# lucidrains/egnn-pytorch

Hardware: AMD Instinct MI355X
Metric: EGNN.forward graphs/sec (higher is better)
Workload: dtype f32; 1 GPU; EGNN(dim=512) masked k-NN (k=32) B=64/GPU N=1024 fp32; graphs_per_gpu=64, nodes=1024, neighbors=32, layers=1, global_batch=64, mask=all-true, parallelism=batch-shard x1 (no data-path collective)

## Files before the change

egnn_pytorch_amd/csrc/edge_pw.hip:

```cpp
#include <type_traits>
#include "egnn_common.h"
#include "egnn_lds_dma.h"

namespace {

typedef _Float16 f16x8 __attribute__((ext_vector_type(8)));
typedef _Float16 f16x4 __attribute__((ext_vector_type(4)));
typedef _Float16 f16x2 __attribute__((ext_vector_type(2)));
typedef float f32x2v __attribute__((ext_vector_type(2)));
typedef uint32_t u32x2 __attribute__((ext_vector_type(2)));
typedef uint32_t u32x4v __attribute__((ext_vector_type(4)));

#ifndef EGNN_PW_WGS
#define EGNN_PW_WGS 5
#endif
#ifndef EGNN_PW_SKIP_MASKED
#define EGNN_PW_SKIP_MASKED 1
#endif
#ifndef EGNN_PW_RESID4
#define EGNN_PW_RESID4 1
#endif

constexpr int PW_THREADS = 256;
constexpr int PW_WAVES = 4;
#ifndef EGNN_PW_EARLY_W
#define EGNN_PW_EARLY_W 1
#endif
#ifndef EGNN_PW_PRIO
#define EGNN_PW_PRIO 0
#endif
#ifndef EGNN_PW_HC
#define EGNN_PW_HC 64
#endif
#ifndef EGNN_PW_ABL
#define EGNN_PW_ABL 0
#endif
constexpr int PW_HC = EGNN_PW_HC;
constexpr int PW_XLD = 32;
constexpr int PW_W2S = 0;
constexpr int PW_WST = PW_W2S + 2 * PW_HC * 64;
constexpr int PW_XCH = PW_WST + 2 * PW_HC * 16;
constexpr int PW_REC = PW_XCH + PW_WAVES * 32 * PW_XLD * 4;
constexpr int PW_SCR = PW_REC + PW_WAVES * 2 * 512;
constexpr int PW_LDS = PW_SCR + PW_WAVES * 256;

__device__ __forceinline__ uint32_t pw_pack_h2(_Float16 a, _Float16 b)
{
    const f16x2 v = {a, b};
    return __builtin_bit_cast(uint32_t, v);
}

template <typename T>
__device__ __forceinline__ T pw_opaque(T v)
{
    asm volatile("" : "+s"(v));
    return v;
}

__device__ __forceinline__ uint32_t lds_addr_of(const void* p)
{
    return __builtin_amdgcn_readfirstlane((uint32_t)(size_t)(__attribute__((address_space(3))) char*)(char*)p);
}

typedef const __attribute__((address_space(4))) egnn_edge_args* pw_args_ptr;
__device__ __forceinline__ pw_args_ptr pw_args()
{
    pw_args_ptr a = (pw_args_ptr)__builtin_amdgcn_kernarg_segment_ptr();
    asm volatile("" : "+s"(a));
    return a;
}

template <bool MULTI>
__global__ __launch_bounds__(PW_THREADS, EGNN_PW_WGS) void edge_pw_kernel(const egnn_edge_args p)
{
    __shared__ __attribute__((aligned(16))) char smem[PW_LDS];

    const int tid = threadIdx.x;
    const int lane = tid & 63;
    const int wave = __builtin_amdgcn_readfirstlane(tid >> 6);
    const int e = lane & 15;
    const int g = lane >> 4;
    const int N = p.N, K = p.K;
    const int R = MULTI ? (K >> 5) : 1;
    const int T = p.B * N;

    const int ngroups = (T + PW_WAVES - 1) / PW_WAVES;
    const int nper = (int)(gridDim.x >> 3);
    const int xcd = (int)(blockIdx.x & 7), wi = (int)(blockIdx.x >> 3);
    const int gq = ngroups >> 3, grem = ngroups & 7;
    const int gstart = xcd * gq + (xcd < grem ? xcd : grem);
    const int gcount = gq + (xcd < grem ? 1 : 0);
    if (wi >= gcount) return;
    const int mygroups = (gcount - wi + nper - 1) / nper;
    const int total_rounds = mygroups * R;

    _Float16* const w2s = reinterpret_cast<_Float16*>(smem + PW_W2S);
    char* const wst = smem + PW_WST;
    float* const xch = reinterpret_cast<float*>(smem + PW_XCH) + wave * (32 * PW_XLD);
    char* const recb = smem + PW_REC + wave * 1024;
    float* const scr = reinterpret_cast<float*>(smem + PW_SCR) + wave * 64;
    const uint32_t xch_lds = lds_addr_of(xch);
    const uint32_t rec_lds = lds_addr_of(recb);

    const int Hp = p.Hp;
    const int nchunks = (Hp + PW_HC - 1) / PW_HC;
#if defined(EGNN_PW_NO_HALF_TAIL) && EGNN_PW_NO_HALF_TAIL
    const bool half_tail = false;
#else
    const bool half_tail = Hp - p.H >= 16;
#endif

    const char* const w2h_g = reinterpret_cast<const char*>(p.W2h);
    const char* const wst_g = reinterpret_cast<const char*>(p.Wst);
    const uint32_t lane16 = (uint32_t)lane * 16u;
    auto stage = [&](int c, int slot) {
        const int c0s = c * PW_HC;
        const int hcs = (Hp - c0s) < PW_HC ? (Hp - c0s) : PW_HC;
        const char* src = w2h_g + (size_t)c0s * 64;
        char* dst = reinterpret_cast<char*>(w2s) + slot * (PW_HC * 64);
        for (int pc = wave; pc < hcs / 16; pc += PW_WAVES) lds_dma16_s(src + pc * 1024, lane16, dst + pc * 1024);
        if (wave == 0) {
            const int tbytes = hcs * 16;
            for (int o = 0; o < tbytes; o += 1024)
                if ((int)lane16 + o < tbytes) lds_dma16_s(wst_g + (size_t)c0s * 16 + o, lane16, wst + slot * (PW_HC * 16) + o);
        }
    };
    auto rec_dma = [&](int tau, int r, int buf) {
        const pw_args_ptr a = pw_args();
        const u32x4s slot_words = make_rsrc_words(a->slots, (uint32_t)((size_t)a->B * a->N * a->K * 16));
        const uint32_t soff = ((uint32_t)tau * (uint32_t)a->K + 32u * (uint32_t)r) * 16u;
        if (lane < 32) gather_dma16(slot_words, (uint32_t)lane * 16u, soff, rec_lds + (uint32_t)buf * 512u);
    };
    auto node_of = [&](int kg) { return (gstart + wi + kg * nper) * PW_WAVES + wave; };
    int zero_v = 0;
    asm volatile("" : "+v"(zero_v));
    auto row_of = [&](int tau) {
        const pw_args_ptr a = pw_args();
        return a->order ? a->order[tau + zero_v] : tau % a->N;
    };

    const float* xr[2];
#pragma unroll
    for (int hb = 0; hb < 2; ++hb) xr[hb] = xch + e * PW_XLD + 4 * ((4 * hb + g) ^ ((e >> 1) & 7));
    const char* const tl = wst + (e * 4 + (g ^ ((e >> 2) & 2))) * 4;
    constexpr int tstep = 16 * 4 * 4;
#if EGNN_PW_RESID4
    f16x4 neg_identity;
#pragma unroll
    for (int u = 0; u < 4; ++u) neg_identity[u] = ((lane & 3) == u) ? (_Float16)-1.f : (_Float16)0.f;
#else
    f16x4 neg_identity;
#pragma unroll
    for (int u = 0; u < 4; ++u) neg_identity[u] = (e == 4 * g + u) ? (_Float16)-1.f : (_Float16)0.f;
#endif
#if defined(EGNN_PW_STAGGER) && EGNN_PW_STAGGER
    for (int q = 0; q < ((wi / 32) % EGNN_PW_WGS) * EGNN_PW_STAGGER; ++q) __builtin_amdgcn_s_sleep(127);
#endif
    stage(0, 0);
    int tau_next = node_of(0);
    bool live_next = tau_next < T;
    if (!live_next) tau_next = T - 1;
    rec_dma(tau_next, 0, 0);
    int i_next_v = row_of(tau_next);
    int ring = 0;

    f32x4 nms = f32x4{0.f, 0.f, 0.f, 0.f};
    float ncs[4] = {0.f, 0.f, 0.f, 0.f};

    int kg = 0, r = 0;
    for (int rho = 0; rho < total_rounds; ++rho) {
        const pw_args_ptr pa = pw_args();
        const int64_t ldp = pa->ldp;
        const int tau = tau_next;
        const bool live = live_next;
        const int b = tau / N;
        const size_t bN = (size_t)b * N;
        const int i = __builtin_amdgcn_readfirstlane(i_next_v);
        const uint32_t prow_bytes = (uint32_t)((size_t)N * ldp * 4);
        const __amdgpu_buffer_rsrc_t pi_rsrc = __builtin_amdgcn_make_buffer_rsrc(const_cast<float*>(pa->Pi + bN * ldp), 0, prow_bytes, 0x00020000);
        const u32x4s pj_words = make_rsrc_words(pa->Pj + bN * ldp, prow_bytes);
        const int cur = rho & 1;
        const char* const rb = recb + cur * 512;

        asm volatile("s_waitcnt vmcnt(0)" ::: "memory");
        __builtin_amdgcn_wave_barrier();
        uint32_t goff[4];
#pragma unroll
        for (int qq = 0; qq < 4; ++qq) {
            const uint32_t j2 = *reinterpret_cast<const uint32_t*>(rb + (8 * qq + (lane >> 3)) * 16) & 0x3fffffffu;
            const uint32_t gchunk = (uint32_t)(((lane & 7) ^ ((4 * qq + (lane >> 4)) & 7)) * 16);
            goff[qq] = (uint32_t)((size_t)j2 * ldp * 4) + gchunk;
        }
        u32x4v rec[2];
#pragma unroll
        for (int t = 0; t < 2; ++t) rec[t] = *reinterpret_cast<const u32x4v*>(rb + (16 * t + e) * 16);
#pragma unroll
        for (int qq = 0; qq < 4; ++qq) gather_dma16(pj_words, goff[qq], 0u, xch_lds + qq * 1024);
        const uint32_t piw = (uint32_t)(((size_t)i * ldp + e) * 4);
        uint32_t piv[2];
        piv[0] = buf_load1(pi_rsrc, piw, 0);
        piv[1] = buf_load1(pi_rsrc, piw, 64);
        if (rho + 1 < total_rounds) {
            if (r + 1 == R) {
                tau_next = node_of(kg + 1);
                live_next = tau_next < T;
                if (!live_next) tau_next = T - 1;
                i_next_v = row_of(tau_next);
                rec_dma(tau_next, 0, cur ^ 1);
            } else {
                rec_dma(tau, r + 1, cur ^ 1);
            }
        }

        u32x2 bq[2];
        bool fm[2];
        const int gq_ = g + pw_opaque(0);
        const uint32_t gm0 = gq_ == 0 ? 0xffffffffu : 0u, gm1 = gq_ == 1 ? 0xffffffffu : 0u, gm2 = gq_ == 2 ? 0xffffffffu : 0u;
#pragma unroll
        for (int t = 0; t < 2; ++t) {
            const uint32_t r0 = rec[t][0], r1 = rec[t][1], r2 = rec[t][2], r3 = rec[t][3];
            const float d = egnn_sqdist_rel(__uint_as_float(r1), __uint_as_float(r2), __uint_as_float(r3));
            float val = d * pa->ws_inv_scale;
            egnn_flag_range(pa->status, live && fabsf(val) >= 6.0e7f && fabsf(val) < __builtin_inff(), EGNN_RANGE_SCALAR);
            if (fabsf(val) >= 6.0e7f) val = __builtin_nanf("");
            const _Float16 s1 = (_Float16)(val * (1.0f / 1024.0f));
            const float rem = val - (float)s1 * 1024.0f;
            const _Float16 rh = (_Float16)rem;
            const _Float16 rl = (_Float16)(rem - (float)rh);
            u32x2 bw;
            bw[0] = 0x3c003c00u & gm0;
            bw[1] = (pw_pack_h2(s1, s1) & gm0) | (pw_pack_h2(rh, rh) & gm1) | (pw_pack_h2(rl, (_Float16)0.f) & gm2);
            bq[t] = bw;
            fm[t] = live && (r0 >> 31) != 0u;
        }

        f32x4 acc[2];
#pragma unroll
        for (int t = 0; t < 2; ++t) acc[t] = f32x4{0.f, 0.f, 0.f, 0.f};
#if EGNN_PW_SKIP_MASKED
        const bool skip_round = pa->U_out == nullptr && __builtin_amdgcn_ballot_w64(fm[0] || fm[1]) == 0ull;
        const bool skip_group = skip_round && ((__builtin_amdgcn_readfirstlane(*reinterpret_cast<const int*>(rb)) >> 30) & 1) != 0;
#else
        constexpr bool skip_round = false, skip_group = false;
#endif

        const bool last_round = rho + 1 == total_rounds;
        auto step = [&](auto half_tag, const int c, const int st, const int slot, const int hoff, const _Float16* w2c, const char* tlc) {
            constexpr bool HALF = decltype(half_tag)::value;
            constexpr int NHB = HALF ? 1 : 2;
            const bool more = hoff + 32 < Hp;
            const int hnext = more ? hoff + 32 : hoff;
            f32x4 x[2][2];
            uint32_t pivn[2];
#if EGNN_PW_EARLY_W
            u32x2 a0[2];
#pragma unroll
            for (int hb = 0; hb < NHB; ++hb)
                a0[hb] = u32x2{0u, *reinterpret_cast<const uint32_t*>(tlc + st * 2 * tstep + hb * tstep)};
            const f16x8 whi = *reinterpret_cast<const f16x8*>(w2c + ((st * 2 + 0) * 64 + lane) * 8);
            const f16x8 wlo = *reinterpret_cast<const f16x8*>(w2c + ((st * 2 + 1) * 64 + lane) * 8);
#endif
#if EGNN_PW_ABL & 2
#pragma unroll
            for (int t = 0; t < 2; ++t)
#pragma unroll
                for (int hb = 0; hb < NHB; ++hb) { x[t][hb] = acc[t] * 0.25f; asm volatile("" : "+v"(x[t][hb])); }
#else
            asm volatile("" ::: "memory");
            __builtin_amdgcn_s_waitcnt(0x0F70);
            asm volatile("" ::: "memory");
            __builtin_amdgcn_wave_barrier();
#pragma unroll
            for (int t = 0; t < 2; ++t)
#pragma unroll
                for (int hb = 0; hb < NHB; ++hb) x[t][hb] = *reinterpret_cast<const f32x4*>(xr[hb] + t * 16 * PW_XLD);
            asm volatile("" ::: "memory");
            __builtin_amdgcn_s_waitcnt(0xC07F);
            asm volatile("" ::: "memory");
            __builtin_amdgcn_wave_barrier();
#endif
            if (!HALF) {
#if EGNN_PW_ABL & 256
                pivn[0] = piv[0]; pivn[1] = piv[1];
#else
                pivn[0] = buf_load1(pi_rsrc, piw, hnext * 4);
                pivn[1] = buf_load1(pi_rsrc, piw, hnext * 4 + 64);
#endif
            }
#if !(EGNN_PW_ABL & 128)
            if (st == 0) {
                if (c + 1 < nchunks) stage(c + 1, slot ^ 1);
                else if (!last_round) stage(0, slot ^ 1);
            }
#endif
#if !(EGNN_PW_ABL & 1)
            if (more) {
#pragma unroll
                for (int qq = 0; qq < 4; ++qq) gather_dma16(pj_words, goff[qq], (uint32_t)(hnext * 4), xch_lds + qq * 1024);
            }
#endif

#if EGNN_PW_EARLY_W
#pragma unroll
            for (int hb = 0; hb < NHB; ++hb) a0[hb][0] = piv[hb];
#else
            u32x2 a0[2];
#pragma unroll
            for (int hb = 0; hb < NHB; ++hb)
                a0[hb] = u32x2{piv[hb], *reinterpret_cast<const uint32_t*>(tlc + st * 2 * tstep + hb * tstep)};
            const f16x8 whi = *reinterpret_cast<const f16x8*>(w2c + ((st * 2 + 0) * 64 + lane) * 8);
            const f16x8 wlo = *reinterpret_cast<const f16x8*>(w2c + ((st * 2 + 1) * 64 + lane) * 8);
#endif
            if (!HALF) {
                piv[0] = pivn[0];
                piv[1] = pivn[1];
            }
#pragma unroll
            for (int t = 0; t < 2; ++t)
#pragma unroll
                for (int hb = 0; hb < NHB; ++hb) {
#if EGNN_PW_ABL & 4
                    asm volatile("" :: "v"(a0[hb]), "v"(bq[t]));
#else
                    x[t][hb] = __builtin_amdgcn_mfma_f32_16x16x16f16(__builtin_bit_cast(f16x4, a0[hb]), __builtin_bit_cast(f16x4, bq[t]), x[t][hb], 0, 0, 0);
#endif
                }
#pragma unroll
            for (int t = 0; t < 2; ++t) {
                f16x8 bhi, blo;
#pragma unroll
                for (int u = 0; u < 8; ++u) { bhi[u] = (_Float16)0.f; blo[u] = (_Float16)0.f; }
#pragma unroll
                for (int hb = 0; hb < NHB; ++hb) {
                    f32x4 a4;
#pragma unroll
                    for (int u = 0; u < 4; ++u) {
                        const float y = x[t][hb][u];
#if EGNN_PW_ABL & 32
                        float h = y;
#else
                        float h = y * __builtin_amdgcn_rcpf(1.0f + __builtin_amdgcn_exp2f(y));
#endif
                        asm("" : "+v"(h));
                        a4[u] = h;
                    }
#if EGNN_PW_ABL & 512
                    const f16x2 h01 = __builtin_bit_cast(f16x2, a4[0]), h23 = __builtin_bit_cast(f16x2, a4[2]);
#else
                    const f16x2 h01 = __builtin_convertvector((f32x2v){a4[0], a4[1]}, f16x2);
                    const f16x2 h23 = __builtin_convertvector((f32x2v){a4[2], a4[3]}, f16x2);
#endif
                    const f16x4 hi4 = {h01[0], h01[1], h23[0], h23[1]};
#if EGNN_PW_ABL & 8
                    const f32x4 l4 = a4;
                    asm volatile("" :: "v"(neg_identity));
#elif EGNN_PW_RESID4
                    const f32x4 l4 = __builtin_amdgcn_mfma_f32_4x4x4f16(neg_identity, hi4, a4, 0, 0, 0);
#else
                    const f32x4 l4 = __builtin_amdgcn_mfma_f32_16x16x16f16(neg_identity, hi4, a4, 0, 0, 0);
#endif
#if EGNN_PW_ABL & 512
                    const f16x2 l01 = __builtin_bit_cast(f16x2, l4[1]), l23 = __builtin_bit_cast(f16x2, l4[3]);
#else
                    const f16x2 l01 = __builtin_bit_cast(f16x2, __builtin_amdgcn_cvt_pkrtz(l4[0], l4[1]));
                    const f16x2 l23 = __builtin_bit_cast(f16x2, __builtin_amdgcn_cvt_pkrtz(l4[2], l4[3]));
#endif
                    bhi[4 * hb + 0] = h01[0]; bhi[4 * hb + 1] = h01[1]; bhi[4 * hb + 2] = h23[0]; bhi[4 * hb + 3] = h23[1];
                    blo[4 * hb + 0] = l01[0]; blo[4 * hb + 1] = l01[1]; blo[4 * hb + 2] = l23[0]; blo[4 * hb + 3] = l23[1];
                }
#if EGNN_PW_ABL & 16
                f32x4 at = acc[t];
                asm volatile("" : "+v"(at) : "v"(whi), "v"(wlo), "v"(bhi), "v"(blo));
                acc[t] = at;
#else
                acc[t] = __builtin_amdgcn_mfma_f32_16x16x32_f16(whi, bhi, acc[t], 0, 0, 0);
                acc[t] = __builtin_amdgcn_mfma_f32_16x16x32_f16(wlo, bhi, acc[t], 0, 0, 0);
                acc[t] = __builtin_amdgcn_mfma_f32_16x16x32_f16(whi, blo, acc[t], 0, 0, 0);
#endif
            }
        };
#if EGNN_PW_PRIO == 1
        asm volatile("s_setprio 0");
#elif EGNN_PW_PRIO == 2
        asm volatile("s_setprio 3");
#endif
        if (skip_group) {
        } else if (skip_round) {
            for (int c = 0; c < nchunks; ++c, ++ring) {
                const int slot = ring & 1;
#if !(EGNN_PW_ABL & 128)
                asm volatile("s_waitcnt vmcnt(0)" ::: "memory");
                __syncthreads();
                if (c + 1 < nchunks) stage(c + 1, slot ^ 1);
                else if (!last_round) stage(0, slot ^ 1);
#endif
            }
        } else
        for (int c = 0; c < nchunks; ++c, ++ring) {
            const int slot = ring & 1;
            const int c0 = c * PW_HC;
            const int hc = (Hp - c0) < PW_HC ? (Hp - c0) : PW_HC;
#if !(EGNN_PW_ABL & 128)
            asm volatile("s_waitcnt vmcnt(0)" ::: "memory");
            __syncthreads();
#endif
            const _Float16* w2c = w2s + slot * (PW_HC * 32);
            const char* tlc = tl + slot * (PW_HC * 16);
            const int nst = hc >> 5;
            for (int st = 0; st < nst; ++st) {
                const int hoff = c0 + st * 32;
                if (half_tail && hoff + 32 >= Hp) step(std::true_type{}, c, st, slot, hoff, w2c, tlc);
                else step(std::false_type{}, c, st, slot, hoff, w2c, tlc);
            }
        }

#if EGNN_PW_PRIO == 1
        asm volatile("s_setprio 3");
#elif EGNN_PW_PRIO == 2
        asm volatile("s_setprio 0");
#endif
        const pw_args_ptr pe = pw_args();
        const bool has_mask = pe->mask != nullptr;
        int32_t* const status = pe->status;
        const float* const gate_w = pe->gate_w;
        const float* const coors_scale = pe->coors_scale;
        if (skip_round) {
            if (!MULTI) {
                nms = f32x4{0.f, 0.f, 0.f, 0.f};
#pragma unroll
                for (int c = 0; c < 4; ++c) ncs[c] = 0.f;
            }
        } else {
        f32x4 b2r, gwr = f32x4{0.f, 0.f, 0.f, 0.f};
        float gb = 0.f;
        const int g4 = pw_opaque(4) * g;
        b2r = *reinterpret_cast<const f32x4*>(pe->b2 + g4);
        if (gate_w) {
            gwr = *reinterpret_cast<const f32x4*>(gate_w + g4);
            gb = pe->gate_b[0];
        }
        float cscale = 0.f;
        if (coors_scale) cscale = coors_scale[0];
        const float w2_inv_scale = pe->w2_inv_scale;
        float* const u_out = pe->U_out;

        float cw[2];
#pragma unroll
        for (int t = 0; t < 2; ++t) {
            f32x4 m;
            bool bad = false;
            f32x4 uu;
#pragma unroll
            for (int u = 0; u < 4; ++u) {
                bad = bad || !(fabsf(acc[t][u]) < __builtin_inff());
                uu[u] = acc[t][u] * w2_inv_scale + b2r[u];
                m[u] = egnn_silu(uu[u]);
            }
            if (u_out && live) *reinterpret_cast<f32x4*>(u_out + ((bN + i) * (size_t)K + 32 * r + 16 * t + e) * 16 + g4) = uu;
            float part = gwr[0] * m[0] + gwr[1] * m[1] + gwr[2] * m[2] + gwr[3] * m[3];
            egnn_flag_range(status, bad && fm[t], EGNN_RANGE_HIDDEN);
            if (gate_w) {
                part = egnn_column_sum4(part, scr, lane);
                const float gt = egnn_sigmoid(part + gb);
                m *= gt;
            }
            acc[t] = m;
            cw[t] = 0.f;
        }

#if EGNN_PW_ABL & 64
        const _Float16* const w3h = nullptr;
#else
        const _Float16* const w3h = static_cast<const _Float16*>(pe->W3h);
#endif
        if (w3h) {
            float part[2] = {0.f, 0.f};
            f16x4 mhi[2], mlo[2];
#pragma unroll
            for (int t = 0; t < 2; ++t) {
                bool bad = false;
#pragma unroll
                for (int u = 0; u < 4; ++u) bad = bad || egnn_beyond_f16(acc[t][u]);
                egnn_flag_range(status, bad && fm[t], EGNN_RANGE_MESSAGE);
#pragma unroll
                for (int u = 0; u < 4; ++u) {
                    const _Float16 h = (_Float16)acc[t][u];
                    mhi[t][u] = h;
                    mlo[t][u] = (_Float16)(acc[t][u] - (float)h);
                }
            }
            constexpr int W3LD = 16, W3IMG = 64 * 16;
            const int w3o = e * W3LD + g4;
            const float* const b3p = pe->b3;
            const float* const w4p = pe->W4;
            const float w3_inv_scale = pe->w3_inv_scale;
            const float clampv = pe->clamp;
#pragma unroll
            for (int blk = 0; blk < 4; ++blk) {
                const f32x4 b3 = *reinterpret_cast<const f32x4*>(b3p + 16 * blk + g4);
                const f32x4 w4 = *reinterpret_cast<const f32x4*>(w4p + 16 * blk + g4);
                const f16x4 w3hi = *reinterpret_cast<const f16x4*>(w3h + 16 * blk * W3LD + w3o);
                const f16x4 w3lo = *reinterpret_cast<const f16x4*>(w3h + W3IMG + 16 * blk * W3LD + w3o);
#pragma unroll
                for (int t = 0; t < 2; ++t) {
                    f32x4 a2 = f32x4{0.f, 0.f, 0.f, 0.f};
                    a2 = __builtin_amdgcn_mfma_f32_16x16x16f16(w3hi, mhi[t], a2, 0, 0, 0);
                    a2 = __builtin_amdgcn_mfma_f32_16x16x16f16(w3lo, mhi[t], a2, 0, 0, 0);
                    a2 = __builtin_amdgcn_mfma_f32_16x16x16f16(w3hi, mlo[t], a2, 0, 0, 0);
#pragma unroll
                    for (int u = 0; u < 4; ++u) part[t] += w4[u] * egnn_silu(a2[u] * w3_inv_scale + b3[u]);
                }
            }
            const float b4 = pe->b4[0];
#pragma unroll
            for (int t = 0; t < 2; ++t) {
                float s = egnn_column_sum4(part[t], scr, lane);
                s += b4;
                if (has_mask && !fm[t]) s = 0.f;
                if (clampv >= 0.f) s = fminf(fmaxf(s, -clampv), clampv);
                if (!fm[t] && !has_mask) s = 0.f;
                cw[t] = s;
            }
        }

        float rn[2][3], keep[2];
#pragma unroll
        for (int t = 0; t < 2; ++t) {
            const u32x4v rc = *reinterpret_cast<const u32x4v*>(rb + (16 * t + e) * 16);
            const uint32_t rw[3] = {rc[1], rc[2], rc[3]};
            float rel[3];
#pragma unroll
            for (int c = 0; c < 3; ++c) rel[c] = __uint_as_float(rw[c]);
            keep[t] = fm[t] ? 1.f : 0.f;
            float inv = 1.f;
            if (coors_scale) {
                float n2 = 0.f;
#pragma unroll
                for (int c = 0; c < 3; ++c) n2 = __builtin_fmaf(rel[c], rel[c], n2);
                inv = cscale / fmaxf(sqrtf(n2), 1e-8f);
            }
#pragma unroll
            for (int c = 0; c < 3; ++c) rn[t][c] = rel[c] * inv;
        }
        const f32x4 zero4 = f32x4{0.f, 0.f, 0.f, 0.f};
        f32x4 ms = (fm[0] ? acc[0] : zero4) + (fm[1] ? acc[1] : zero4);
        float cs[4];
#pragma unroll
        for (int c = 0; c < 3; ++c) cs[c] = __builtin_fmaf(cw[1], rn[1][c], cw[0] * rn[0][c]);
        cs[3] = keep[0] + keep[1];
#pragma unroll
        for (int u = 0; u < 4; ++u) ms[u] = egnn_row16_sum(ms[u]);
#pragma unroll
        for (int c = 0; c < 4; ++c) cs[c] = egnn_row16_sum(cs[c]);
        if (MULTI) {
#pragma unroll
            for (int u = 0; u < 4; ++u) nms[u] += ms[u];
#pragma unroll
            for (int c = 0; c < 4; ++c) ncs[c] += cs[c];
        } else {
#pragma unroll
            for (int u = 0; u < 4; ++u) nms[u] = 0.f + ms[u];
#pragma unroll
            for (int c = 0; c < 4; ++c) ncs[c] = 0.f + cs[c];
        }
        }

        if (r + 1 == R) {
            if (live) {
                const size_t row = bN + i;
                const int m_dim = pe->m_dim;
                float* const m_i = pe->m_i;
                _Float16* const node_hi = static_cast<_Float16*>(pe->node_hi);
                _Float16* const node_lo = static_cast<_Float16*>(pe->node_lo);
                const int dim = pe->dim;
                if (e == 0 && node_hi && !m_i && (dim & 3) == 0 && m_dim == 16) {
                    const int gch = pw_opaque(4) * g;
                    const int pool_mean = pe->pool_mean, nkt = pe->node_kp / 16;
                    f32x4 val;
                    bool bad = false;
#pragma unroll
                    for (int u = 0; u < 4; ++u) {
                        float v = 0.f + nms[u];
                        if (pool_mean) {
                            if (has_mask) {
                                const float cnt = 0.f + ncs[3];
                                v = (cnt == 0.f) ? 0.f : v / fmaxf(cnt, 1e-8f);
                            } else {
                                v = v / (float)K;
                            }
                        }
                        bad = bad || egnn_beyond_f16(v);
                        val[u] = v;
                    }
                    egnn_flag_range(status, bad, EGNN_RANGE_MESSAGE);
                    f16x4 h4, l4;
#pragma unroll
                    for (int u = 0; u < 4; ++u) {
                        h4[u] = (_Float16)val[u];
                        l4[u] = (_Float16)(val[u] - (float)h4[u]);
                    }
                    const size_t off = egnn_pk_off((int64_t)row, dim + gch, nkt);
                    *reinterpret_cast<f16x4*>(node_hi + off) = h4;
                    *reinterpret_cast<f16x4*>(node_lo + off) = l4;
                } else if (e == 0 && (m_i || node_hi)) {
                    const int gch = pw_opaque(4) * g;
                    const int pool_mean = pe->pool_mean, nkt = pe->node_kp / 16;
#pragma unroll
                    for (int u = 0; u < 4; ++u) {
                        const int ch = gch + u;
                        float val = 0.f + nms[u];
                        if (ch < m_dim) {
                            if (pool_mean) {
                                if (has_mask) {
                                    const float cnt = 0.f + ncs[3];
                                    val = (cnt == 0.f) ? 0.f : val / fmaxf(cnt, 1e-8f);
                                } else {
                                    val = val / (float)K;
                                }
                            }
                            if (m_i) m_i[row * m_dim + ch] = val;
                            if (node_hi) {
                                egnn_flag_range(status, egnn_beyond_f16(val), EGNN_RANGE_MESSAGE);
                                const _Float16 h = (_Float16)val;
                                const size_t off = egnn_pk_off((int64_t)row, dim + ch, nkt);
                                node_hi[off] = h;
                                node_lo[off] = (_Float16)(val - (float)h);
                            }
                        }
                    }
                }
                float* const coors_out = pe->coors_out;
                if (lane < 3 && coors_out) {
                    const float val = 0.f + (lane == 0 ? ncs[0] : (lane == 1 ? ncs[1] : ncs[2]));
                    coors_out[row * 3 + lane] = pe->coors[row * 3 + lane] + val;
                }
            }
            if (MULTI) {
                nms = f32x4{0.f, 0.f, 0.f, 0.f};
#pragma unroll
                for (int c = 0; c < 4; ++c) ncs[c] = 0.f;
            }
            r = 0;
            ++kg;
        } else {
            ++r;
        }
    }
    asm volatile("s_waitcnt vmcnt(0)" ::: "memory");
}

}

extern "C" int egnn_edge_pw_covers(int B, int N, int K, int S, int fourier, int edge_dim, int m_dim, int coor_dim, int64_t ldp)
{
    if (coor_dim != 3 || K < 32 || (K % 32) != 0 || K > 4096) return 0;
    if (S != 1 || fourier != 0 || edge_dim != 0 || m_dim > 16) return 0;
    if ((int64_t)B * N * K * 16 > 0xffffffffLL) return 0;
    if ((int64_t)N * ldp * 4 > 0xffffffffLL) return 0;
    return 1;
}

int egnn_edge_pw_launch(const egnn_edge_args* args, void* stream)
{
    const egnn_edge_args& a = *args;
    if (!egnn_edge_pw_covers(a.B, a.N, a.K, a.S, a.fourier, a.edge_dim, a.m_dim, a.coor_dim, a.ldp) || a.wst_terms != 4) return EGNN_E_UNSUPPORTED;
    if (!a.slots || !a.pi_split || (!a.idx && a.K != a.N)) return EGNN_E_UNSUPPORTED;
    if (a.drop_thr) return EGNN_E_UNSUPPORTED;
    int dev = 0, cus = 0;
    if (hipGetDevice(&dev) != hipSuccess || hipDeviceGetAttribute(&cus, hipDeviceAttributeMultiprocessorCount, dev) != hipSuccess || cus <= 0)
        return (int)hipGetLastError();
    const int64_t T = (int64_t)a.B * a.N;
    const int64_t ngroups = (T + PW_WAVES - 1) / PW_WAVES;
#if defined(EGNN_PW_GRID_MULT)
    int64_t grid = (int64_t)cus * EGNN_PW_WGS * EGNN_PW_GRID_MULT;
    if (grid > ngroups) grid = ngroups;
#else
    int64_t grid = ngroups;
#endif
    grid = (grid + 7) / 8 * 8;
    if (a.K == 32) hipLaunchKernelGGL(edge_pw_kernel<false>, dim3((unsigned)grid), dim3(PW_THREADS), 0, static_cast<hipStream_t>(stream), a);
    else hipLaunchKernelGGL(edge_pw_kernel<true>, dim3((unsigned)grid), dim3(PW_THREADS), 0, static_cast<hipStream_t>(stream), a);
    return egnn_launch_status();
}
```

Before: 25120 graphs/s.

## Alias edge-record buffer into exchange LDS to raise occupancy to six workgroups

Removes the per-wave double-buffered record and scratch LDS regions and reuses the xch exchange area for both, which shrinks LDS per workgroup. With that, launch bounds rise from 5 to 6 workgroups per CU. Since the record buffer is now overwritten by the neighbor gathers, the prefetch of the next record moves to the epilogue, and the epilogue re-reads the relative-coordinate record from global memory. The prefetch now overlaps less with compute, and the epilogue does extra global loads and waits, which may cost latency and register pressure.

Result: faster. 25470 graphs/s, median of 6 (+1.4%).

```diff
diff --git a/egnn_pytorch_amd/csrc/edge_pw.hip b/egnn_pytorch_amd/csrc/edge_pw.hip
--- a/egnn_pytorch_amd/csrc/edge_pw.hip
+++ b/egnn_pytorch_amd/csrc/edge_pw.hip
@@ -12,7 +12,7 @@
 typedef uint32_t u32x4v __attribute__((ext_vector_type(4)));
 
 #ifndef EGNN_PW_WGS
-#define EGNN_PW_WGS 5
+#define EGNN_PW_WGS 6
 #endif
 #ifndef EGNN_PW_SKIP_MASKED
 #define EGNN_PW_SKIP_MASKED 1
@@ -40,9 +40,8 @@
 constexpr int PW_W2S = 0;
 constexpr int PW_WST = PW_W2S + 2 * PW_HC * 64;
 constexpr int PW_XCH = PW_WST + 2 * PW_HC * 16;
-constexpr int PW_REC = PW_XCH + PW_WAVES * 32 * PW_XLD * 4;
-constexpr int PW_SCR = PW_REC + PW_WAVES * 2 * 512;
-constexpr int PW_LDS = PW_SCR + PW_WAVES * 256;
+constexpr int PW_LDS = PW_XCH + PW_WAVES * 32 * PW_XLD * 4;
+constexpr int PW_XCH_SCR = 512;
 
 __device__ __forceinline__ uint32_t pw_pack_h2(_Float16 a, _Float16 b)
 {
@@ -60,6 +59,12 @@
 __device__ __forceinline__ uint32_t lds_addr_of(const void* p)
 {
     return __builtin_amdgcn_readfirstlane((uint32_t)(size_t)(__attribute__((address_space(3))) char*)(char*)p);
+}
+
+__device__ __forceinline__ void pw_gather_dma16(u32x4s rsrc, uint32_t voff, uint32_t soff, uint32_t lds_base, int lds_imm)
+{
+    asm volatile("s_add_u32 m0, %3, %4\n\ts_nop 0\n\tbuffer_load_dwordx4 %0, %1, %2 offen lds"
+                 :: "v"(voff), "s"(rsrc), "s"(soff), "s"(lds_base), "i"(lds_imm) : "memory", "m0", "scc");
 }
 
 typedef const __attribute__((address_space(4))) egnn_edge_args* pw_args_ptr;
@@ -97,10 +102,9 @@
     _Float16* const w2s = reinterpret_cast<_Float16*>(smem + PW_W2S);
     char* const wst = smem + PW_WST;
     float* const xch = reinterpret_cast<float*>(smem + PW_XCH) + wave * (32 * PW_XLD);
-    char* const recb = smem + PW_REC + wave * 1024;
-    float* const scr = reinterpret_cast<float*>(smem + PW_SCR) + wave * 64;
+    const char* const rb = reinterpret_cast<const char*>(xch);
+    float* const scr = xch + PW_XCH_SCR / 4;
     const uint32_t xch_lds = lds_addr_of(xch);
-    const uint32_t rec_lds = lds_addr_of(recb);
 
     const int Hp = p.Hp;
     const int nchunks = (Hp + PW_HC - 1) / PW_HC;
@@ -125,11 +129,11 @@
                 if ((int)lane16 + o < tbytes) lds_dma16_s(wst_g + (size_t)c0s * 16 + o, lane16, wst + slot * (PW_HC * 16) + o);
         }
     };
-    auto rec_dma = [&](int tau, int r, int buf) {
+    auto rec_dma = [&](int tau, int r, int lane_x) {
         const pw_args_ptr a = pw_args();
         const u32x4s slot_words = make_rsrc_words(a->slots, (uint32_t)((size_t)a->B * a->N * a->K * 16));
         const uint32_t soff = ((uint32_t)tau * (uint32_t)a->K + 32u * (uint32_t)r) * 16u;
-        if (lane < 32) gather_dma16(slot_words, (uint32_t)lane * 16u, soff, rec_lds + (uint32_t)buf * 512u);
+        if (lane_x < 32) gather_dma16(slot_words, (uint32_t)lane_x * 16u, soff, xch_lds);
     };
     auto node_of = [&](int kg) { return (gstart + wi + kg * nper) * PW_WAVES + wave; };
     int zero_v = 0;
@@ -160,7 +164,7 @@
     int tau_next = node_of(0);
     bool live_next = tau_next < T;
     if (!live_next) tau_next = T - 1;
-    rec_dma(tau_next, 0, 0);
+    rec_dma(tau_next, 0, lane);
     int i_next_v = row_of(tau_next);
     int ring = 0;
 
@@ -171,50 +175,42 @@
     for (int rho = 0; rho < total_rounds; ++rho) {
         const pw_args_ptr pa = pw_args();
         const int64_t ldp = pa->ldp;
+        const int lane_s = (lane + pw_opaque(0)) & 63;
+        const int e_s = lane_s & 15, g_s = lane_s >> 4;
         const int tau = tau_next;
         const bool live = live_next;
-        const int b = tau / N;
-        const size_t bN = (size_t)b * N;
+        const int Ns = pa->N;
+        const int b = tau / Ns;
+        const size_t bN = (size_t)b * Ns;
         const int i = __builtin_amdgcn_readfirstlane(i_next_v);
-        const uint32_t prow_bytes = (uint32_t)((size_t)N * ldp * 4);
+        const uint32_t prow_bytes = (uint32_t)((size_t)Ns * ldp * 4);
         const __amdgpu_buffer_rsrc_t pi_rsrc = __builtin_amdgcn_make_buffer_rsrc(const_cast<float*>(pa->Pi + bN * ldp), 0, prow_bytes, 0x00020000);
         const u32x4s pj_words = make_rsrc_words(pa->Pj + bN * ldp, prow_bytes);
-        const int cur = rho & 1;
-        const char* const rb = recb + cur * 512;
 
         asm volatile("s_waitcnt vmcnt(0)" ::: "memory");
         __builtin_amdgcn_wave_barrier();
         uint32_t goff[4];
 #pragma unroll
         for (int qq = 0; qq < 4; ++qq) {
-            const uint32_t j2 = *reinterpret_cast<const uint32_t*>(rb + (8 * qq + (lane >> 3)) * 16) & 0x3fffffffu;
-            const uint32_t gchunk = (uint32_t)(((lane & 7) ^ ((4 * qq + (lane >> 4)) & 7)) * 16);
+            const uint32_t j2 = *reinterpret_cast<const uint32_t*>(rb + (8 * qq + (lane_s >> 3)) * 16) & 0x3fffffffu;
+            const uint32_t gchunk = (uint32_t)(((lane_s & 7) ^ ((4 * qq + g_s) & 7)) * 16);
             goff[qq] = (uint32_t)((size_t)j2 * ldp * 4) + gchunk;
         }
         u32x4v rec[2];
 #pragma unroll
-        for (int t = 0; t < 2; ++t) rec[t] = *reinterpret_cast<const u32x4v*>(rb + (16 * t + e) * 16);
-#pragma unroll
-        for (int qq = 0; qq < 4; ++qq) gather_dma16(pj_words, goff[qq], 0u, xch_lds + qq * 1024);
-        const uint32_t piw = (uint32_t)(((size_t)i * ldp + e) * 4);
+        for (int t = 0; t < 2; ++t) rec[t] = *reinterpret_cast<const u32x4v*>(rb + (16 * t + e_s) * 16);
+        asm volatile("s_waitcnt lgkmcnt(0)" ::: "memory");
+        __builtin_amdgcn_wave_barrier();
+#pragma unroll
+        for (int qq = 0; qq < 4; ++qq) pw_gather_dma16(pj_words, goff[qq], 0u, xch_lds, qq * 1024);
+        const uint32_t piw = (uint32_t)(((size_t)i * ldp + e_s) * 4);
         uint32_t piv[2];
         piv[0] = buf_load1(pi_rsrc, piw, 0);
         piv[1] = buf_load1(pi_rsrc, piw, 64);
-        if (rho + 1 < total_rounds) {
-            if (r + 1 == R) {
-                tau_next = node_of(kg + 1);
-                live_next = tau_next < T;
-                if (!live_next) tau_next = T - 1;
-                i_next_v = row_of(tau_next);
-                rec_dma(tau_next, 0, cur ^ 1);
-            } else {
-                rec_dma(tau, r + 1, cur ^ 1);
-            }
-        }
 
         u32x2 bq[2];
         bool fm[2];
-        const int gq_ = g + pw_opaque(0);
+        const int gq_ = g_s;
         const uint32_t gm0 = gq_ == 0 ? 0xffffffffu : 0u, gm1 = gq_ == 1 ? 0xffffffffu : 0u, gm2 = gq_ == 2 ? 0xffffffffu : 0u;
 #pragma unroll
         for (int t = 0; t < 2; ++t) {
@@ -239,7 +235,7 @@
         for (int t = 0; t < 2; ++t) acc[t] = f32x4{0.f, 0.f, 0.f, 0.f};
 #if EGNN_PW_SKIP_MASKED
         const bool skip_round = pa->U_out == nullptr && __builtin_amdgcn_ballot_w64(fm[0] || fm[1]) == 0ull;
-        const bool skip_group = skip_round && ((__builtin_amdgcn_readfirstlane(*reinterpret_cast<const int*>(rb)) >> 30) & 1) != 0;
+        const bool skip_group = skip_round && ((__builtin_amdgcn_readfirstlane((int)rec[0][0]) >> 30) & 1) != 0;
 #else
         constexpr bool skip_round = false, skip_group = false;
 #endif
@@ -296,7 +292,7 @@
 #if !(EGNN_PW_ABL & 1)
             if (more) {
 #pragma unroll
-                for (int qq = 0; qq < 4; ++qq) gather_dma16(pj_words, goff[qq], (uint32_t)(hnext * 4), xch_lds + qq * 1024);
+                for (int qq = 0; qq < 4; ++qq) pw_gather_dma16(pj_words, goff[qq], (uint32_t)(hnext * 4), xch_lds, qq * 1024);
             }
 #endif
 
@@ -420,7 +416,22 @@
         asm volatile("s_setprio 0");
 #endif
         const pw_args_ptr pe = pw_args();
+        const int lane_e = (lane + pw_opaque(0)) & 63;
+        const int e_e = lane_e & 15, g_e = lane_e >> 4;
         const bool has_mask = pe->mask != nullptr;
+        const int Ke = pe->K;
+        if (skip_round) asm volatile("s_waitcnt vmcnt(0)" ::: "memory");
+        if (rho + 1 < total_rounds) {
+            if (r + 1 == R) {
+                tau_next = node_of(kg + 1);
+                live_next = tau_next < T;
+                if (!live_next) tau_next = T - 1;
+                i_next_v = row_of(tau_next);
+                rec_dma(tau_next, 0, lane_e);
+            } else {
+                rec_dma(tau, r + 1, lane_e);
+            }
+        }
         int32_t* const status = pe->status;
         const float* const gate_w = pe->gate_w;
         const float* const coors_scale = pe->coors_scale;
@@ -431,9 +442,15 @@
                 for (int c = 0; c < 4; ++c) ncs[c] = 0.f;
             }
         } else {
+        const __amdgpu_buffer_rsrc_t rec_rsrc = __builtin_amdgcn_make_buffer_rsrc(
+            const_cast<void*>(static_cast<const void*>(pe->slots)), 0, (uint32_t)((size_t)pe->B * pe->N * Ke * 16), 0x00020000);
+        const uint32_t rec_soff = ((uint32_t)tau * (uint32_t)Ke + 32u * (uint32_t)r) * 16u;
+        f32x4 rcv[2];
+#pragma unroll
+        for (int t = 0; t < 2; ++t) rcv[t] = buf_load4(rec_rsrc, (uint32_t)e_e * 16u, (int)(rec_soff + 256u * t));
         f32x4 b2r, gwr = f32x4{0.f, 0.f, 0.f, 0.f};
         float gb = 0.f;
-        const int g4 = pw_opaque(4) * g;
+        const int g4 = 4 * g_e;
         b2r = *reinterpret_cast<const f32x4*>(pe->b2 + g4);
         if (gate_w) {
             gwr = *reinterpret_cast<const f32x4*>(gate_w + g4);
@@ -456,11 +473,11 @@
                 uu[u] = acc[t][u] * w2_inv_scale + b2r[u];
                 m[u] = egnn_silu(uu[u]);
             }
-            if (u_out && live) *reinterpret_cast<f32x4*>(u_out + ((bN + i) * (size_t)K + 32 * r + 16 * t + e) * 16 + g4) = uu;
+            if (u_out && live) *reinterpret_cast<f32x4*>(u_out + ((bN + i) * (size_t)Ke + 32 * r + 16 * t + e_e) * 16 + g4) = uu;
             float part = gwr[0] * m[0] + gwr[1] * m[1] + gwr[2] * m[2] + gwr[3] * m[3];
             egnn_flag_range(status, bad && fm[t], EGNN_RANGE_HIDDEN);
             if (gate_w) {
-                part = egnn_column_sum4(part, scr, lane);
+                part = egnn_column_sum4(part, scr, lane_e);
                 const float gt = egnn_sigmoid(part + gb);
                 m *= gt;
             }
@@ -490,7 +507,7 @@
                 }
             }
             constexpr int W3LD = 16, W3IMG = 64 * 16;
-            const int w3o = e * W3LD + g4;
+            const int w3o = e_e * W3LD + g4;
             const float* const b3p = pe->b3;
             const float* const w4p = pe->W4;
             const float w3_inv_scale = pe->w3_inv_scale;
@@ -514,7 +531,7 @@
             const float b4 = pe->b4[0];
 #pragma unroll
             for (int t = 0; t < 2; ++t) {
-                float s = egnn_column_sum4(part[t], scr, lane);
+                float s = egnn_column_sum4(part[t], scr, lane_e);
                 s += b4;
                 if (has_mask && !fm[t]) s = 0.f;
                 if (clampv >= 0.f) s = fminf(fmaxf(s, -clampv), clampv);
@@ -526,11 +543,7 @@
         float rn[2][3], keep[2];
 #pragma unroll
         for (int t = 0; t < 2; ++t) {
-            const u32x4v rc = *reinterpret_cast<const u32x4v*>(rb + (16 * t + e) * 16);
-            const uint32_t rw[3] = {rc[1], rc[2], rc[3]};
-            float rel[3];
-#pragma unroll
-            for (int c = 0; c < 3; ++c) rel[c] = __uint_as_float(rw[c]);
+            const float rel[3] = {rcv[t][1], rcv[t][2], rcv[t][3]};
             keep[t] = fm[t] ? 1.f : 0.f;
             float inv = 1.f;
             if (coors_scale) {
@@ -573,8 +586,8 @@
                 _Float16* const node_hi = static_cast<_Float16*>(pe->node_hi);
                 _Float16* const node_lo = static_cast<_Float16*>(pe->node_lo);
                 const int dim = pe->dim;
-                if (e == 0 && node_hi && !m_i && (dim & 3) == 0 && m_dim == 16) {
-                    const int gch = pw_opaque(4) * g;
+                if (e_e == 0 && node_hi && !m_i && (dim & 3) == 0 && m_dim == 16) {
+                    const int gch = 4 * g_e;
                     const int pool_mean = pe->pool_mean, nkt = pe->node_kp / 16;
                     f32x4 val;
                     bool bad = false;
@@ -586,7 +599,7 @@
                                 const float cnt = 0.f + ncs[3];
                                 v = (cnt == 0.f) ? 0.f : v / fmaxf(cnt, 1e-8f);
                             } else {
-                                v = v / (float)K;
+                                v = v / (float)Ke;
                             }
                         }
                         bad = bad || egnn_beyond_f16(v);
@@ -602,8 +615,8 @@
                     const size_t off = egnn_pk_off((int64_t)row, dim + gch, nkt);
                     *reinterpret_cast<f16x4*>(node_hi + off) = h4;
                     *reinterpret_cast<f16x4*>(node_lo + off) = l4;
-                } else if (e == 0 && (m_i || node_hi)) {
-                    const int gch = pw_opaque(4) * g;
+                } else if (e_e == 0 && (m_i || node_hi)) {
+                    const int gch = 4 * g_e;
                     const int pool_mean = pe->pool_mean, nkt = pe->node_kp / 16;
 #pragma unroll
                     for (int u = 0; u < 4; ++u) {
@@ -615,7 +628,7 @@
                                     const float cnt = 0.f + ncs[3];
                                     val = (cnt == 0.f) ? 0.f : val / fmaxf(cnt, 1e-8f);
                                 } else {
-                                    val = val / (float)K;
+                                    val = val / (float)Ke;
                                 }
                             }
                             if (m_i) m_i[row * m_dim + ch] = val;
@@ -630,9 +643,9 @@
                     }
                 }
                 float* const coors_out = pe->coors_out;
-                if (lane < 3 && coors_out) {
-                    const float val = 0.f + (lane == 0 ? ncs[0] : (lane == 1 ? ncs[1] : ncs[2]));
-                    coors_out[row * 3 + lane] = pe->coors[row * 3 + lane] + val;
+                if (lane_e < 3 && coors_out) {
+                    const float val = 0.f + (lane_e == 0 ? ncs[0] : (lane_e == 1 ? ncs[1] : ncs[2]));
+                    coors_out[row * 3 + lane_e] = pe->coors[row * 3 + lane_e] + val;
                 }
             }
             if (MULTI) {
```
